# serval/kaboodle

Hardware: AMD Instinct MI355X
Metric: simulated peer-rounds/sec (whole node) + rounds to fingerprint convergence (higher is better)
Workload: dtype u8

## Files before the change

### include/kaboodle_sim.h

```cpp
#ifndef KABOODLE_SIM_H
#define KABOODLE_SIM_H

#include <stddef.h>
#include <stdint.h>

#ifdef __cplusplus
extern "C" {
#endif

#define KB_ABI_VERSION 3u

enum {
  KB_OK = 0,
  KB_INVALID_OPERATION = 1,
  KB_IO_ERROR = 2,
  KB_NO_DEVICE = 3,
  KB_STOPPING_FAILED = 4,
  KB_INVALID_ARGUMENT = 5,
  KB_CAPACITY = 6
};

enum { KB_INIT_JOIN = 0,
       KB_INIT_CONVERGED = 1 };

enum { KB_FAILED_SIM_SENDER = 0,
       KB_FAILED_SOCKET_FAITHFUL = 1 };

typedef struct kb_config {
  uint32_t abi_version;
  uint32_t capacity;
  uint32_t initial_nodes;
  uint32_t init_mode;
  uint64_t seed;
  uint32_t loss_threshold;
  uint32_t churn_threshold;
  int32_t  fault_end_round;
  uint32_t max_waves;
  uint32_t failed_mode;
  uint32_t id_len;
  uint32_t partition_groups;
  int32_t  partition_start;
  int32_t  partition_end;
  int32_t  device;
  uint32_t debug_flags;
  uint32_t track_latency;
  uint32_t variant;
  uint32_t sparse_row_cap;
  uint32_t stat_flags;
  uint32_t reserved[1];
} kb_config;
enum { KB_STAT_NO_SF_FAILED_DROPS = 1u };
enum { KB_VARIANT_SAME_WINDOW_BCAST = 1u,
       KB_VARIANT_EXACT_LRU = 2u,
       KB_VARIANT_SPARSE_ROWS = 4u };

enum {
  KB_DBG_PHASEB_HBM = 1u,
  KB_DBG_RESP_HBM = 2u,
  KB_DBG_KP_HBM = 4u,
  KB_DBG_KP_BIG_SMALL = 8u,
  KB_DBG_PROC_UNSORTED = 16u,
  KB_DBG_WAVE_GRAPH = 32u,
  KB_DBG_RESP_WAVE_HBM = 64u,
  KB_DBG_NO_UNION = 128u,
  KB_DBG_A3X_KPL8 = 256u,
  KB_DBG_A3X_WIDE = 512u,
  KB_DBG_WAVE0_SERIAL = 1024u,
  KB_DBG_RESP_SERIAL = 2048u
};

enum { KB_STATE_KNOWN = 0, KB_STATE_WAITING_FOR_PING = 1, KB_STATE_WAITING_FOR_INDIRECT_PING = 2 };
typedef struct kb_peer_state {
  uint32_t peer;
  uint32_t state;
  int32_t  since;
  uint32_t latency_ms;
  uint32_t identity_len;
  uint8_t  identity[32];
} kb_peer_state;
#define KB_LATENCY_NONE 0xFFFFFFFFu

typedef struct kb_stats {
  int32_t  round;
  uint32_t alive;
  uint32_t agree;
  int32_t  first_converged_round;
  int32_t  last_converged_round;
  uint32_t next_free_id;
  uint64_t sent_ping, sent_ping_req, sent_ack, sent_known_peers, sent_kpr;
  uint64_t bcast_join, bcast_failed;
  uint64_t drop_dead, drop_loss, drop_window, drop_oversize, drop_partition, drop_bcast;
  uint64_t removed_timeout, removed_failed, join_responses, curious_overflow, churn_leaves, churn_joins;
  uint64_t sent_kp_ids;
  uint64_t alive_rounds;
  uint64_t probe_responses;
  uint64_t exported;
  uint64_t reserved[4];
} kb_stats;

typedef struct kb_sim kb_sim;

void kb_config_default(kb_config* cfg);

int  kb_sim_create(const kb_config* cfg, kb_sim** out);
int  kb_sim_destroy(kb_sim* sim);
int  kb_sim_step(kb_sim* sim, uint32_t rounds);

int  kb_sim_start_node(kb_sim* sim, uint32_t node);
int  kb_sim_stop_node(kb_sim* sim, uint32_t node);
int  kb_sim_restart_node(kb_sim* sim, uint32_t node, uint32_t* new_node);
int  kb_sim_is_running(kb_sim* sim, uint32_t node, int* running);
int  kb_sim_ping_addrs(kb_sim* sim, uint32_t node, const uint32_t* peers, size_t n);
int  kb_sim_set_identity(kb_sim* sim, uint32_t node, const uint8_t* identity, size_t len);
int  kb_sim_identity(kb_sim* sim, uint32_t node, uint8_t* buf, size_t cap, size_t* len);

int  kb_sim_fingerprint(kb_sim* sim, uint32_t node, uint32_t* fp);
int  kb_sim_fingerprints(kb_sim* sim, uint32_t* fps, size_t cap);
int  kb_sim_peers(kb_sim* sim, uint32_t node, uint32_t* peers, size_t cap, size_t* n);
int  kb_sim_peer_states(kb_sim* sim, uint32_t node, kb_peer_state* out, size_t cap, size_t* n);
int  kb_sim_stats(kb_sim* sim, kb_stats* out);
int  kb_sim_true_fingerprint(kb_sim* sim, uint32_t* fp);
// ... 112 lines not shown
```

### kaboodle_amd/_ffi.py

```python
from __future__ import annotations

import ctypes as C
import os
from dataclasses import dataclass

KB_ABI_VERSION = 3
KB_OK, KB_INVALID_OPERATION, KB_IO_ERROR, KB_NO_DEVICE, KB_STOPPING_FAILED, KB_INVALID_ARGUMENT, KB_CAPACITY = range(7)
KB_INIT_JOIN, KB_INIT_CONVERGED = 0, 1
KB_FAILED_SIM_SENDER, KB_FAILED_SOCKET_FAITHFUL = 0, 1
KB_DBG_PHASEB_HBM, KB_DBG_RESP_HBM, KB_DBG_KP_HBM, KB_DBG_KP_BIG_SMALL, KB_DBG_PROC_UNSORTED = 1, 2, 4, 8, 16
KB_DBG_ALL = 31
KB_DBG_WAVE_GRAPH = 32
KB_DBG_RESP_WAVE_HBM = 64
KB_DBG_NO_UNION = 128
KB_DBG_A3X_KPL8 = 256
KB_DBG_A3X_WIDE = 512
KB_DBG_WAVE0_SERIAL = 1024
KB_DBG_RESP_SERIAL = 2048
KB_VARIANT_SAME_WINDOW_BCAST, KB_VARIANT_EXACT_LRU = 1, 2
KB_STAT_NO_SF_FAILED_DROPS = 1
KB_VARIANT_SPARSE_ROWS = 4
KB_LATENCY_NONE = 0xFFFFFFFF
KT_ROWPASS, KT_ROUND, KT_FOLD, KT_RESP, KT_PROC = 0, 1, 2, 3, 4
KB_WAVE_SLOTS = 9
STATE_NAMES = {0: "Known", 1: "WaitingForPing", 2: "WaitingForIndirectPing"}


class KbConfig(C.Structure):
    _fields_ = [
        ("abi_version", C.c_uint32), ("capacity", C.c_uint32), ("initial_nodes", C.c_uint32),
        ("init_mode", C.c_uint32), ("seed", C.c_uint64), ("loss_threshold", C.c_uint32),
        ("churn_threshold", C.c_uint32), ("fault_end_round", C.c_int32), ("max_waves", C.c_uint32),
        ("failed_mode", C.c_uint32), ("id_len", C.c_uint32), ("partition_groups", C.c_uint32),
        ("partition_start", C.c_int32), ("partition_end", C.c_int32), ("device", C.c_int32),
        ("debug_flags", C.c_uint32), ("track_latency", C.c_uint32), ("variant", C.c_uint32),
        ("sparse_row_cap", C.c_uint32), ("stat_flags", C.c_uint32), ("reserved", C.c_uint32 * 1),
    ]


class KbPeerState(C.Structure):
    _fields_ = [("peer", C.c_uint32), ("state", C.c_uint32), ("since", C.c_int32), ("latency_ms", C.c_uint32),
                ("identity_len", C.c_uint32), ("identity", C.c_uint8 * 32)]


PEER_STATE_DTYPE = [("peer", "<u4"), ("state", "<u4"), ("since", "<i4"), ("latency_ms", "<u4"), ("identity_len", "<u4"),
                    ("identity", "u1", (32,))]


class KbStats(C.Structure):
    _fields_ = [
        ("round", C.c_int32), ("alive", C.c_uint32), ("agree", C.c_uint32),
        ("first_converged_round", C.c_int32), ("last_converged_round", C.c_int32), ("next_free_id", C.c_uint32),
        ("sent_ping", C.c_uint64), ("sent_ping_req", C.c_uint64), ("sent_ack", C.c_uint64),
        ("sent_known_peers", C.c_uint64), ("sent_kpr", C.c_uint64),
        ("bcast_join", C.c_uint64), ("bcast_failed", C.c_uint64),
        ("drop_dead", C.c_uint64), ("drop_loss", C.c_uint64), ("drop_window", C.c_uint64),
        ("drop_oversize", C.c_uint64), ("drop_partition", C.c_uint64), ("drop_bcast", C.c_uint64),
        ("removed_timeout", C.c_uint64), ("removed_failed", C.c_uint64), ("join_responses", C.c_uint64),
        ("curious_overflow", C.c_uint64), ("churn_leaves", C.c_uint64), ("churn_joins", C.c_uint64),
        ("sent_kp_ids", C.c_uint64), ("alive_rounds", C.c_uint64), ("probe_responses", C.c_uint64),
        ("exported", C.c_uint64), ("reserved", C.c_uint64 * 4),
    ]

    def as_dict(self) -> dict:
        return {n: getattr(self, n) for n, _ in self._fields_ if n != "reserved"}


class KbKernelTime(C.Structure):
    _fields_ = [("name", C.c_char * 24), ("ms", C.c_double), ("launches", C.c_uint64), ("bytes", C.c_uint64),
                ("has_bytes", C.c_uint32), ("pad", C.c_uint32), ("wave_ms", C.c_double * KB_WAVE_SLOTS)]

# ... 927 lines not shown
```

### kaboodle_amd/csrc/kb_common.h

```cpp
#pragma once
#include "kb_device.h"
#include "../../include/kaboodle_sim.h"

namespace kb {

enum StatIdx {
  S_PING, S_PINGREQ, S_ACK, S_KP, S_KPR, S_BJOIN, S_BFAIL, S_DEAD, S_LOSS, S_WINDOW, S_OVERSIZE, S_PART, S_BDROP,
  S_RMTIMEOUT, S_RMFAILED, S_JRESP, S_CUROVF, S_CLEAVE, S_CJOIN,
  S_KPIDS,
  S_ROWB,
  S_FOLDB,
  S_A3ROWS, S_A3DEEP, S_A3CHUNKS,
  S_ALIVER,
  S_RESPB,
  S_PROCB,
  S_PROBERESP,
  S_EXPORT,
  S_A3X32, S_A3XCLAMP, S_A3XFEW, S_A3XLIVE, S_A3XWIDE,
  NSTAT
};
enum CtrIdx {
  C_KP, C_SLOW, C_ACTIVE, C_AGREE, C_ALIVE, C_LEAVES, C_NEXTFREE, C_ERR, C_FIRSTCONV, C_LASTCONV, C_LASTAGREE,
  C_LASTALIVE, C_DBG_INS, C_DBG_FP, C_DBG_MAXFP,
  C_DBG_KPR, C_DBG_KPRLOG, C_DBG_BASE,
  C_DBG_TNODE, C_DBG_TMAX, C_DBG_TBASE, C_DBG_TINS,
  C_DBG_TSTART, C_DBG_TEND, C_DBG_MSGS,
  C_TICK,
  C_ROUND,
  C_PATHS,
  C_DBG_SLOW_LONG, C_DBG_SLOW_NONMEM, C_DBG_SLOW_DIRTY, C_DBG_SLOW_KPR, C_DBG_SLOW_OTHER,
  C_RESTN,
  C_XREC, C_XPAY,
  NCTR
};
enum : uint32_t { PATH_PHASEB_HBM = 1, PATH_RESP_SCRATCH_SAMPLED = 2, PATH_RESP_SCRATCH_FULL = 4, PATH_KP_BIG_HBM = 8,
                  PATH_PROC_UNSORTED = 16, PATH_BFAIL_PREP_HBM = 32, PATH_RESP_WAVE = 64, PATH_KP_BIG_LDS = 128,
                  PATH_RESP_WAVE_HBM = 256,
                  PATH_PROC_DEFERRED = 512,
                  PATH_ROWPASS_LDS_HBM_LISTS = 1024,
                  PATH_KPR_WRAPPED = 2048,
                  PATH_RESP_JOINERS_HBM = 4096,
                  PATH_JOIN_LIST_PAST_UCAP = 8192,
                  PATH_RESP_PHASE1 = 16384,
                  PATH_A2_RESPONDER = 32768 };
constexpr int NSEG = 64;
constexpr int ZT = 9;
constexpr int ZB = 9 * 1024;

struct Dev {
  uint32_t lo, hi;
  uint32_t C, W, SEGW, NWR;
  uint32_t segq, segm;
  uint32_t k0, k1;
  uint32_t loss_thr, churn_thr;
  int32_t fault_end;
  uint32_t failed_mode;
  uint32_t pgroups;
  int32_t pstart, pend;
  uint32_t uniform, L;
  uint32_t capk, capj;
  uint32_t paybound;
  uint32_t dbg;
  uint32_t dev;
  uint8_t* stamp;
  uint32_t* bits;
  uint2* segp;
  unsigned long long* sdirty;
  uint8_t* dirty;
  uint8_t* alive;
  uint8_t* idset;
  uint32_t* abits;
  int32_t* start_round;
  uint32_t* n;
  uint32_t* fp;
  int32_t* last_bcast;
  uint32_t* a3cur;
  Susp* susp;
  Cur* cur;
  uint32_t* paq;
  uint32_t* paq_n;
  uint32_t* cseg;
  uint32_t* segmul;
  uint32_t* seglen;
  uint32_t* zpow;
  uint32_t* zfin;
// ... 379 lines not shown
```

### kaboodle_amd/csrc/kb_sim.hip

```cpp
#include <hip/hip_runtime.h>
#include <hip/hip_ext.h>
#include <stdint.h>
#include <stdio.h>
#include <string.h>
#include <stdlib.h>
#include <string>
#include <vector>
#include <array>
#include <algorithm>
#include <atomic>
#include <thread>
#include "kb_common.h"
#include "kb_wire.h"
#include "kb_round.h"
#include "kb_tick.h"
#include "kb_waves.h"
#include "kb_xfer.h"
#include "kb_sparse.h"

using namespace kb;

enum KId : int {
  KI_REBASE, KI_EVENTS, KI_CHURN_LEAVE, KI_CHURN_JOIN, KI_ALIVE_BITS, KI_TRUEFP_PART, KI_TRUEFP_FIN, KI_LOG_MARK,
  KI_LAT_MARK, KI_BFAIL_PREP, KI_ROWPASS, KI_LAT_SWEEP, KI_SCAN_TILES, KI_SCAN_APPLY, KI_SET_CAP, KI_RESP_WAVE,
// ... 266 lines not shown

struct kb_sim {
  kb_config cfg;
  SpSim* sp = nullptr;
  Dev d;
  int device;
  hipStream_t st;
  hipStream_t st2 = nullptr;
  hipStream_t st3 = nullptr;
  hipEvent_t ev_fork[5] = {nullptr, nullptr, nullptr, nullptr, nullptr}, ev_join[5] = {nullptr, nullptr, nullptr, nullptr, nullptr};
  uint32_t C, W, S;
  uint32_t lo, hi, R;
  int rank, world;
  Xfer* xf;
  bool in_group;
  std::vector<void*> allocs;
  int32_t round;
  bool probed = false;
  std::vector<uint8_t> h_ident, h_idlen;
  std::vector<uint8_t> h_pend; std::vector<int16_t> h_pendlen;
  std::vector<uint8_t> h_moved;
  std::vector<uint8_t> h_idset;
  std::vector<uint8_t> h_ext;
  size_t n_ext = 0;
  std::vector<XRec> inj; std::vector<uint32_t> inj_ids;
  std::vector<uint32_t> inj_join;
  XRec* d_inj = nullptr; uint32_t* d_inj_ids = nullptr; size_t d_inj_cap = 0, d_inj_ids_cap = 0;
  std::vector<kb_unicast> xq; std::vector<uint32_t> xq_ids;
  std::vector<Event> events;
  uint32_t* rpack = nullptr; uint32_t* rpack_in = nullptr;
  std::vector<kb_wire_addr> probe_q, probes;
  std::vector<kb_probe_response> presp;
  uint2* d_presp = nullptr; uint32_t* d_presp_n = nullptr; size_t presp_cap = 0;
  OutBuf ob[2];
  WaveCtl wc;
  uint32_t msg_cap, pay_cap;
  BCast* bfail; BCast* bjoin;
  BCast* bfail_loc; BCast* bjoin_loc;
  uint32_t nf, nj;
  uint32_t ucap = 0;
  uint32_t host_paths = 0;
  uint64_t xbytes_cross = 0, xbytes_all = 0;
  BcastSlots bs;
  uint32_t* join_off; uint32_t* fail_off;
  uint32_t* scan_tot; uint32_t* scan_tiles;
  unsigned long long* newmask; unsigned long long* respmask; size_t mask_words;
  unsigned long long* newmask_base; unsigned long long* respmask_base;
  uint32_t* nresp; uint32_t* paysum; uint32_t* nbase; uint32_t* resp_off;
  uint32_t* resp_nodes; uint32_t* bf_gid; uint8_t* bf_dep;
  uint32_t* slow;
  uint32_t* rest[2] = {nullptr, nullptr};
  uint32_t* rest2n = nullptr;
  uint8_t* a2flag = nullptr;
  uint32_t* defer = nullptr;
  uint32_t* w0ctr = nullptr;
  uint16_t* lat_col;
  uint32_t* fnamed;
  uint32_t* resp_scratch; size_t resp_scratch_words;
  RowOut ro;
  Event* d_events; size_t events_cap;
  XState xs;
  uint32_t* xall; unsigned long long* xstats;
  std::vector<uint32_t> h_xall;
  Msg* rmsg; uint32_t* rpay; uint8_t* rstatus; uint32_t* rinbox; uint32_t* rkp;
  size_t rmsg_cap, rpay_cap;
  double round_ms;
  uint32_t* rr = nullptr;
  uint64_t round_launches, bj_total, bf_total;
  struct KRec { int16_t kid, wave; hipEvent_t a, b; };
  int prof_level = 1;
  bool capturing = false;
  int cur_wave = -1;
  std::vector<hipEvent_t> ev_free;
  std::vector<KRec> krec;
  double k_ms[NKI] = {};
  double k_wms[NKI][KB_WAVE_SLOTS] = {};
  uint64_t k_n[NKI] = {};
  uint64_t k_bytes0[NSTAT] = {};
  uint64_t host_syncs = 0;
  uint32_t ncu = 256;
  uint32_t* cs_buf = nullptr;
  uint32_t* rc_buf = nullptr;
  uint2* rc_pairs = nullptr; size_t rc_pairs_cap = 0;
  char* fc_buf = nullptr; size_t fc_cap = 0;
  double census_ms[CM_N] = {};
  bool debug_waves = false;
  size_t lds_per_cu = 65536;
  std::vector<kb_sim*> shards;
  LocalHub* hub;
  std::vector<uint32_t> watch_node, watch_fp;
  std::vector<uint32_t*> watch_snap;
  uint32_t* ev_out = nullptr;
  uint32_t* h_pin = nullptr;
  uint32_t* d_pin = nullptr;
  uint32_t pin_seq = 0;
  uint64_t occ_key = ~0ull; int occ_val = 0;
  bool graph_on = false;
  hipGraph_t wave_graph = nullptr; hipGraphExec_t wave_exec = nullptr;
  uint64_t buf_gen = 0, wave_gen = ~0ull;
  uint32_t* lc_buf = nullptr;
  double sn_ms = 0;
  uint32_t* dl_base = nullptr;
  uint8_t* dl_run = nullptr;
  int32_t dl_round = 0;
  uint32_t* dl_buf = nullptr;
  uint32_t* is_buf = nullptr;
// ... 220 lines not shown
constexpr uint32_t KB_FOLD_WAVES = 16384;
  while (S < 64 && groups * S < KB_FOLD_WAVES) S <<= 1;
  s->S = S;
  Dev& d = s->d;
  d.lo = s->lo; d.hi = s->hi;
  d.C = C; d.W = W; d.SEGW = W / NSEG; d.NWR = W / 32;
  d.segq = d.SEGW / 128;
  d.segm = d.segq > 1 ? (uint32_t)(((1ull << 32) + d.segq - 1) / d.segq) : 0u;
  d.k0 = (uint32_t)cfg->seed; d.k1 = (uint32_t)(cfg->seed >> 32);
  d.loss_thr = cfg->loss_threshold; d.churn_thr = cfg->churn_threshold; d.fault_end = cfg->fault_end_round;
  d.failed_mode = cfg->failed_mode; d.pgroups = cfg->partition_groups; d.pstart = cfg->partition_start;
  d.pend = cfg->partition_end;
  const uint32_t Lid = cfg->id_len;
  d.capk = (BUFSZ - 20 - Lid) / (18 + Lid);
  d.capj = (BUFSZ - 20 - Lid - 1) / (18 + Lid);
  d.paybound = C < d.capk ? C : d.capk;
  d.dbg = cfg->debug_flags;
  if (const char* dv = getenv("KB_DEV")) d.dev = (uint32_t)atoi(dv);
  s->debug_waves = getenv("KB_DEBUG_WAVES") != nullptr;
  if (const char* gv = getenv("KB_WAVE_GRAPH")) s->graph_on = atoi(gv) != 0;
  if (cfg->debug_flags & KB_DBG_WAVE_GRAPH) s->graph_on = true;
  s->h_ident.assign((size_t)C * MAXID, 0); s->h_idlen.assign(C, (uint8_t)Lid);
  s->h_pend.assign((size_t)C * MAXID, 0); s->h_pendlen.assign(C, (int16_t)-1); s->h_moved.assign(C, 0);
  s->h_idset.assign(C, 0);
  for (uint32_t j = 0; j < C; ++j) default_identity(j, Lid, &s->h_ident[(size_t)j * MAXID]);
  hipError_t e = hipSuccess;
#define A(ptr, n) if (e == hipSuccess) e = talloc(s, &(ptr), (n))
#define AR(ptr, n) if (e == hipSuccess) e = ralloc(s, &(ptr), (n))
  AR(d.stamp, W); AR(d.bits, d.NWR); AR(d.segp, NSEG); AR(d.sdirty, 1);
  AR(d.dirty, 1); A(d.alive, C); A(d.idset, C); A(d.ext, C); A(d.abits, d.NWR); A(d.start_round, C); AR(d.n, 1); AR(d.fp, 1);
  AR(d.last_bcast, 1); AR(d.a3cur, 1); AR(d.susp, SLOTS); AR(d.cur, CSLOTS); AR(d.paq, PAQ);
  AR(d.paq_n, 1); A(d.cseg, C); A(d.segmul, C); A(d.seglen, C); A(d.zpow, (size_t)C + 2); A(d.zfin, (size_t)C + 2);
  A(d.ztab, 17 * 128); A(d.zbtab, ZB);
  A(d.htab, (size_t)(W / 8) * 256); A(d.stats, NSTAT); A(d.sacc, (size_t)NACC * NSTAT); A(d.ctr, NCTR); A(d.truefp, 1); A(d.tfpart, TRUEFP_G);
  AR(d.flog, LOGCAP); AR(d.flog_n, 1); AR(d.fstart, 16); AR(d.kpr_big, 1);
  if (cfg->variant == KB_VARIANT_EXACT_LRU) { AR(d.tst, W); AR(d.tlb, W / 1024); }
  if (cfg->track_latency) { A(d.lat, (size_t)W * lat_stride(R)); A(s->lat_col, C); A(s->fnamed, d.NWR); }
  s->msg_cap = std::max<uint32_t>(8u * R + (uint32_t)TICK_MAX * R, 1u << 16);
  s->pay_cap = std::max<uint32_t>((d.capk + 1) * R, 1u << 24);
  for (int b = 0; b < 2; ++b) {
    A(s->ob[b].msgs, s->msg_cap); A(s->ob[b].pay, s->pay_cap); AR(s->ob[b].off, 1); AR(s->ob[b].cap, 1);
    AR(s->ob[b].cnt, 1); AR(s->ob[b].poff, 1);
    s->ob[b].msg_cap = s->msg_cap; s->ob[b].pay_cap = s->pay_cap;
  }
  AR(s->wc.cnt1, 1); AR(s->wc.bnd, 1); AR(s->wc.bpay, 1); AR(s->wc.cursor, 1);
  AR(s->wc.in_off, 1); A(s->wc.active, R);
  AR(s->wc.kcnt, 1); AR(s->wc.kpay, 1); AR(s->wc.kcur, 1); AR(s->wc.koff, 1);
  if (!xf) { A(s->wc.status, s->msg_cap); A(s->wc.inbox, s->msg_cap); A(s->wc.kin, s->msg_cap); }
  A(s->bfail, (size_t)C * SLOTS); A(s->bjoin, C);
  AR(s->bs.join, 1); AR(s->bs.nfail, 1); AR(s->bs.fail, SLOTS); AR(s->join_off, 1); AR(s->fail_off, 1);
  A(s->scan_tot, 32); A(s->rr, 4); A(s->scan_tiles, 5 * ((std::max<size_t>(C, (size_t)world * R) + 1023) / 1024) + 5);
  AR(s->nresp, 1); AR(s->paysum, 1); AR(s->nbase, 1); AR(s->resp_off, 1);
  A(s->resp_nodes, R); A(s->bf_gid, (size_t)C * SLOTS); A(s->bf_dep, (size_t)C * SLOTS); A(s->slow, R); A(s->defer, R); A(s->w0ctr, W0_WORDS);
  A(s->rest[0], R); A(s->rest[1], R); A(s->rest2n, 1); AR(s->a2flag, 1);
  AR(s->ro.part, 10);
  if (xf) {
    XState& x = s->xs;
    x.world = (uint32_t)world; x.R = R; x.S = rows_per; x.RS = R + 1;
    x.NWW = d.NWR; x.nju = 0; x.nj = 0; x.uon = 0;
    s->ucap = std::min<uint32_t>(UCAP, C);
    A(x.ostatus, s->msg_cap); A(x.xcnt, (size_t)world * x.RS); A(x.xpay, (size_t)world * x.RS);
    A(x.xoff, (size_t)world * x.RS); A(x.xpoff, (size_t)world * x.RS); A(x.xb, 2 * world);
    A(x.smsg, (size_t)s->msg_cap + s->ucap); A(x.spay, (size_t)s->pay_cap + (size_t)s->ucap * x.NWW);
    A(x.jslot, C); A(x.ubits, (size_t)s->ucap * x.NWW); A(x.uany, s->ucap);
    A(s->xall, std::max(2 * world * world, 3 * world));
    A(s->xstats, NSTAT);
    A(s->bfail_loc, (size_t)R * SLOTS); A(s->bjoin_loc, R);
    s->h_xall.assign(2 * world * world, 0);
  }
#undef A
#undef AR
  if (e != hipSuccess) { seterr(std::string("device allocation failed: ") + hipGetErrorString(e)); destroy_shard(s); return KB_CAPACITY; }
  (void)hipMemset(L(s, d.kpr_big), 0xFF, 4ull * R);
  if (xf) { (void)hipMemset(s->xs.jslot, 0xFF, 4ull * C); (void)hipMemset(s->xs.ubits, 0, 4ull * s->ucap * s->xs.NWW); }
  if (d.lat) { (void)hipMemset(d.lat, 0xFF, 2ull * lat_stride(R) * W); (void)hipMemset(s->fnamed, 0, 4ull * d.NWR); }
  if (d.tst) {
    (void)hipMemsetD32(d.tst + (size_t)s->lo * W, INT32_MIN / 2, (size_t)R * W);
    (void)hipMemsetD32(d.tlb + (size_t)s->lo * (W / 1024), INT32_MIN, (size_t)R * (W / 1024));
  }
  s->wc.msg_cap = s->msg_cap; s->wc.pay_cap = s->pay_cap;
  if (hipStreamCreateWithFlags(&s->st, hipStreamNonBlocking) != hipSuccess) { destroy_shard(s); seterr("stream"); return KB_IO_ERROR; }
  if (hipStreamCreateWithFlags(&s->st2, hipStreamNonBlocking) != hipSuccess) { destroy_shard(s); seterr("stream"); return KB_IO_ERROR; }
  if (hipStreamCreateWithFlags(&s->st3, hipStreamNonBlocking) != hipSuccess) { destroy_shard(s); seterr("stream"); return KB_IO_ERROR; }
  for (int k = 0; k < 5; ++k)
    if (hipEventCreateWithFlags(&s->ev_fork[k], hipEventDisableTiming) != hipSuccess ||
        hipEventCreateWithFlags(&s->ev_join[k], hipEventDisableTiming) != hipSuccess) { destroy_shard(s); seterr("events"); return KB_IO_ERROR; }
  if (hipHostMalloc((void**)&s->h_pin, 4 * PIN_WORDS, hipHostMallocMapped | hipHostMallocCoherent) != hipSuccess) {
    s->h_pin = nullptr; destroy_shard(s); seterr("pinned buffer"); return KB_IO_ERROR;
  }
  if (hipHostGetDevicePointer((void**)&s->d_pin, s->h_pin, 0) != hipSuccess) { destroy_shard(s); seterr("pinned buffer mapping"); return KB_IO_ERROR; }
  if (const char* pv = getenv("KB_PROF")) s->prof_level = atoi(pv);
  int rc = upload_segments(s);
  if (rc) { destroy_shard(s); return rc; }
  uint32_t ctr0[NCTR] = {0};
  ctr0[C_NEXTFREE] = cfg->initial_nodes;
  ctr0[C_FIRSTCONV] = 0xFFFFFFFFu; ctr0[C_LASTCONV] = 0xFFFFFFFFu;
  if (hipMemcpy(d.ctr, ctr0, sizeof ctr0, hipMemcpyHostToDevice) != hipSuccess) { destroy_shard(s); seterr("ctr upload"); return KB_IO_ERROR; }
  const uint32_t tb = 256, gb = (C + tb - 1) / tb;
  if (cfg->init_mode == KB_INIT_CONVERGED) {
    k_init_converged_rows<<<4096, 256, 0, s->st>>>(d, cfg->initial_nodes);
    k_init_converged_nodes<<<gb, tb, 0, s->st>>>(d, cfg->initial_nodes);
  } else {
    k_init_nodes<<<gb, tb, 0, s->st>>>(d, cfg->initial_nodes);
  }
  if (hipStreamSynchronize(s->st) != hipSuccess) { destroy_shard(s); seterr("init failed"); return KB_IO_ERROR; }
  *out = s;
  return KB_OK;
// ... 489 lines not shown
  const uint32_t R = s->R;
  if (!s->inj_join.empty()) { const int rc = merge_ext_joins(s->st, s->bjoin, &s->nj, s->inj_join, 0, s->C); if (rc) return rc; }
  PhaseB& pb = q.pb;
  pb.bfail = s->bfail; pb.nf = s->nf; pb.bjoin = s->bjoin; pb.nj = s->nj; pb.JW = (s->nj + 63) / 64;
  pb.nresp = s->nresp; pb.paysum = s->paysum; pb.nbase = s->nbase;
  if (pb.JW) {
    const size_t words = (size_t)R * pb.JW;
    if (words > s->mask_words) {
      const int rc = eng_grow_group(s, &s->mask_words, words, words, &s->newmask_base, &s->respmask_base);
      if (rc) return rc;
    }
    s->newmask = bias(s->newmask_base, pb.JW, s->lo);
    s->respmask = bias(s->respmask_base, pb.JW, s->lo);
  }
  pb.newmask = s->newmask; pb.respmask = s->respmask;
  pb.gid = s->bf_gid; pb.dep = s->bf_dep;
  q.lat_fail = d.lat && s->nf && d.failed_mode == KB_FAILED_SIM_SENDER;
  pb.fnamed = q.lat_fail ? s->fnamed : nullptr;
  if (q.lat_fail) klaunch(s, KI_LAT_MARK, k_lat_mark, dim3((s->nf + 255) / 256), dim3(256), 0, (const BCast*)s->bfail, s->nf, s->fnamed);
  const bool pb_hbm = (d.dbg & KB_DBG_PHASEB_HBM) != 0;
  if (s->nf > BFAIL_LDS_MAX || (pb_hbm && s->nf)) klaunch(s, KI_BFAIL_PREP, k_bfail_prep, dim3((s->nf + 255) / 256), dim3(256), 0, (const BCast*)s->bfail, s->nf, s->bf_gid, s->bf_dep, d.ctr + C_PATHS);
  else if (s->nf) klaunch(s, KI_BFAIL_PREP, k_bfail_prep_lds, dim3(1), dim3(1024), 0, (const BCast*)s->bfail, s->nf, s->bf_gid, s->bf_dep);
  { const int rc = dbg_bcast_shape(s, r); if (rc) return rc; }
  {
    const RowPlan p = rowpass_plan(s, pb_hbm);
    { const int rc = dbg_rowpass_begin(s, r, p); if (rc) return rc; }
    if (p.ldsb && !p.ll) s->host_paths |= PATH_ROWPASS_LDS_HBM_LISTS;
    rowpass_with(p, [&](auto k) { klaunch(s, KI_ROWPASS, k, dim3(p.blocks), dim3(64 * p.wpb), (uint32_t)p.lds, d, pb, s->ro, r); });
    { const int rc = dbg_rowpass_shares(s, r, p); if (rc) return rc; }
  }
  side_fork(s, 0);
  klaunch_on(s, s->st2, KI_ALIVE_BITS, k_alive_bits, dim3((d.NWR + TB - 1) / TB), dim3(TB), 0, d);
  klaunch_on(s, s->st2, KI_TRUEFP_PART, k_truefp_part, dim3(TRUEFP_G), dim3(256), 0, d, d.tfpart);
  klaunch_on(s, s->st2, KI_TRUEFP_FIN, k_truefp_fin, dim3(1), dim3(64), 0, d, d.tfpart);
  side_done(s, 0);
  if (q.lat_fail) {
    klaunch_on(s, s->st2, KI_LAT_SWEEP, k_lat_sweep, dim3((lat_stride(R) / 8 + 255) / 256, std::min<uint32_t>(s->nf, 16384)), dim3(256), 0, d,
            (const BCast*)s->bfail, (const uint32_t*)s->bf_gid, s->nf, s->fnamed);
    side_done(s, 1);
  }
  { const int rc = round_take_probes(s, R, &q.np); if (rc) return rc; }
  if (q.np) klaunch(s, KI_PROBE, k_probe, dim3(gnode(s)), dim3(TB), 0, d, q.np, r, s->d_presp, s->d_presp_n, (uint32_t)s->presp_cap);
  return KB_OK;
}

static bool resp_rows_hbm(const kb_sim* s) { return s->W > RESP_LDS_W || (s->d.dbg & KB_DBG_RESP_HBM); }
static int launch_join_responses(kb_sim* s, Round& q, uint32_t resp_nodes, uint32_t phase) {
  Dev& d = s->d;
  const int32_t r = q.r;
  OutBuf& o0 = s->ob[0];
  hipStream_t st = phase == 2 ? s->st3 : s->st;
  uint32_t* rest = s->rest[phase == 2];
  uint32_t* restn = phase == 2 ? s->rest2n : d.ctr + C_RESTN;
  const uint32_t wcap = phase == 1 ? s->ncu : 4096;
  const uint32_t grid = std::min<uint32_t>(resp_nodes, 4096);
  const size_t words = resp_words(d.NWR, s->W / 256);
  uint32_t* scratch = nullptr;
  size_t lds = 4 * words;
  const bool resp_hbm = resp_rows_hbm(s);
  if (resp_hbm) {
    { const int rc = eng_grow(s, &s->resp_scratch, &s->resp_scratch_words, words * grid); if (rc) return rc; }
    scratch = s->resp_scratch;
    lds = 0;
  }
  const size_t wlds = 16ull * rwave_words(d.NWR, s->W / 256);
  const size_t hlds = 4ull * rwave_head(s->W / 256);
  const bool full_on = wlds <= 65536 && !(d.dbg & (KB_DBG_RESP_HBM | KB_DBG_RESP_WAVE_HBM));
  const uint32_t hwaves = (uint32_t)std::min<size_t>(4, 65536 / hlds);
  const bool head_on = !full_on && hwaves >= 1 && !(d.dbg & KB_DBG_RESP_HBM);
  const bool wave_on = full_on || head_on;
  { const int rc = dbg_resp_clear(s); if (rc) return rc; }
  if (full_on) {
    klaunch_on(s, st, KI_RESP_WAVE, k_resp_wave<false>, dim3(std::min<uint32_t>((resp_nodes + 3) / 4, wcap)), dim3(256), (uint32_t)wlds, d,
               q.pb, (const uint32_t*)s->resp_nodes, (const uint32_t*)(s->scan_tot + 4), o0, r, rest, restn, phase, (const uint8_t*)s->a2flag);
  } else if (head_on) {
    klaunch_on(s, st, KI_RESP_WAVE, k_resp_wave<true>, dim3(std::min<uint32_t>((resp_nodes + hwaves - 1) / hwaves, wcap)),
               dim3(64 * hwaves), (uint32_t)(hwaves * hlds), d, q.pb, (const uint32_t*)s->resp_nodes,
               (const uint32_t*)(s->scan_tot + 4), o0, r, rest, restn, phase, (const uint8_t*)s->a2flag);
  }
  klaunch_on(s, st, KI_RESP_NODE, k_resp_node, dim3(wave_on ? std::min<uint32_t>(grid, 2 * s->ncu) : grid), dim3(256), (uint32_t)lds, d, q.pb,
             (const uint32_t*)(wave_on ? rest : s->resp_nodes), (const uint32_t*)(wave_on ? restn : s->scan_tot + 4),
             o0, r, scratch, wave_on, phase, (const uint8_t*)s->a2flag);
  return dbg_resp_report(s, r);
}
static bool resp_overlap_on(const kb_sim* s) {
  return !s->xf && !resp_rows_hbm(s) && !s->debug_waves && !(s->d.dbg & KB_DBG_RESP_SERIAL);
}
static void launch_tick_scan(kb_sim* s, Round& q) {
  klaunch(s, KI_TICK_SCAN, k_tick_scan, dim3(gnode(s)), dim3(TB), 0, s->d, s->bs, q.r, s->slow, s->a2flag);
  q.tick_scanned = true;
}

static int round_wave0_regions(kb_sim* s, Round& q) {
  Dev& d = s->d;
  const int32_t r = q.r;
  const uint32_t R = s->R;
  OutBuf& o0 = s->ob[0];
  q.ninj = (uint32_t)s->inj.size();
  if (q.ninj) {
    if (q.ninj > s->d_inj_cap) { const int rc = eng_grow(s, &s->d_inj, &s->d_inj_cap, 2 * (size_t)q.ninj); if (rc) return rc; }
    if (s->inj_ids.size() > s->d_inj_ids_cap || !s->d_inj_ids) {
      const int rc = eng_grow(s, &s->d_inj_ids, &s->d_inj_ids_cap, 2 * s->inj_ids.size() + 16);
      if (rc) return rc;
    }
    HIPCHK(hipMemcpyAsync(s->d_inj, s->inj.data(), sizeof(XRec) * q.ninj, hipMemcpyHostToDevice, s->st));
    if (!s->inj_ids.empty()) {
      HIPCHK(hipMemcpyAsync(s->d_inj_ids, s->inj_ids.data(), 4 * s->inj_ids.size(), hipMemcpyHostToDevice, s->st));
      q.inj_pay = true;
    }
    klaunch(s, KI_EVENTS, k_inject_prep, dim3(1), dim3(64), 0, d, (const XRec*)s->d_inj, q.ninj, s->paysum);
  }
  {
    ScanArgs a = scan_args(s, R, s->scan_tot);
    a.narr = 3;
    a.in[0] = L(s, s->nresp); a.out[0] = L(s, s->resp_off);
    a.in[1] = L(s, s->paysum); a.out[1] = L(s, o0.poff);
    a.in[2] = L(s, s->nresp); a.out[2] = L(s, o0.off); a.addc[2] = TICK_MAX;
    a.list = s->resp_nodes; a.list_base = s->lo;
    launch_scan(s, a);
  }
  const bool need_tot = s->nj > 0 || q.inj_pay;
  klaunch(s, KI_SET_CAP, k_set_cap, dim3(gnode(s)), dim3(TB), 0, d, s->nresp, o0.cap, o0.cnt, s->scan_tot, s->d_pin, need_tot ? ++s->pin_seq : 0u,
          s->rest2n);
  if (!need_tot) return KB_OK;
  const uint32_t* tot = s->h_pin;
  { const int rc = wait_pin(s, s->pin_seq); if (rc) return rc; }
  const uint32_t pay_tot = tot[1], msg_tot = tot[2], resp_nodes = tot[4];
  if (msg_tot > o0.msg_cap || pay_tot > o0.pay_cap) { const int rc = grow_wave0(s, msg_tot, pay_tot); if (rc) return rc; }
  if (s->n_ext) { const int rc = round_size_exports(s, msg_tot, pay_tot); if (rc) return rc; }
  if (!resp_nodes) return KB_OK;
  if (!resp_overlap_on(s)) return launch_join_responses(s, q, resp_nodes, 0);
  launch_tick_scan(s, q);
  side_fork(s, 4);
  { const int rc = launch_join_responses(s, q, resp_nodes, 2); if (rc) return rc; }
  side_done(s, 4);
  q.resp_side = true;
  return launch_join_responses(s, q, resp_nodes, 1);
}

static int round_tick(kb_sim* s, Round& q) {
  Dev& d = s->d;
  const int32_t r = q.r;
  const uint32_t R = s->R, gn = gnode(s);
  OutBuf& o0 = s->ob[0];
  if (q.lat_fail) side_join(s, 1);
  if (!q.tick_scanned) launch_tick_scan(s, q);
  klaunch(s, KI_TICK_PRE, k_tick_pre, dim3(std::min<uint32_t>((R + 3) / 4, 1024)), dim3(256), 0, d, o0, s->bs, r, s->slow,
          (const uint32_t*)s->nresp);
  if (d.tst) {
    side_fork(s, 2);
    const uint32_t kpl = a3_kpl(s->W, d.dbg);
    if (kpl == 2) klaunch_on(s, s->st2, KI_A3_EXACT, k_a3_exact<2>, dim3((R + 3) / 4), dim3(256), 0, d, s->ro.part, r);
    else if (kpl) klaunch_on(s, s->st2, KI_A3_EXACT, k_a3_exact<A3X_KPL>, dim3((R + 3) / 4), dim3(256), 0, d, s->ro.part, r);
    else klaunch_on(s, s->st2, KI_A3_EXACT, k_a3_exact<0>, dim3((R + 3) / 4), dim3(256), 0, d, s->ro.part, r);
    side_done(s, 2);
  }
  if (d.uniform) klaunch(s, KI_FOLD, k_fold, dim3(((R + 63) / 64 + 3) / 4 * s->S), dim3(256), 0, d, FoldArgs{s->S});
  if (d.uniform) klaunch(s, KI_FP_ROWS, k_fp_rows, dim3((FP_LANES * R + TB - 1) / TB), dim3(TB), 0, d);
  side_join(s, 0);
  if (d.tst) side_join(s, 2);
  if (q.resp_side) side_join(s, 4);
  klaunch(s, KI_TICK_POST, k_tick_post, dim3(gn), dim3(TB), 0, d, s->ro, o0, r);
  if (q.ninj) {
    klaunch(s, KI_EVENTS, k_inject, dim3(1), dim3(64), 0, d, o0, (const XRec*)s->d_inj, q.ninj, (const uint32_t*)s->d_inj_ids);
    s->inj.clear(); s->inj_ids.clear();
  }
  {
    ScanArgs a = scan_args(s, R, s->scan_tot);
    a.narr = 2;
    a.in[0] = L(s, s->bs.join); a.out[0] = L(s, s->join_off);
    a.in[1] = L(s, s->bs.nfail); a.out[1] = L(s, s->fail_off);
    launch_scan(s, a);
  }
  klaunch(s, KI_BCAST_WRITE, k_bcast_write, dim3(gn), dim3(TB), 0, d, s->bs, (const uint32_t*)s->join_off,
          (const uint32_t*)s->fail_off, s->xf ? s->bjoin_loc : s->bjoin, s->xf ? s->bfail_loc : s->bfail);
  return KB_OK;
}

static int round_window(kb_sim* s, Round& q) {
  hipStream_t st = s->st;
  if (s->xf || s->debug_waves || !s->graph_on) return launch_waves(s, q.r);
  if (!s->wave_exec || s->wave_gen != s->buf_gen) {
    if (s->wave_exec) { (void)hipGraphExecDestroy(s->wave_exec); s->wave_exec = nullptr; }
    if (s->wave_graph) { (void)hipGraphDestroy(s->wave_graph); s->wave_graph = nullptr; }
    HIPCHK(hipStreamBeginCapture(st, hipStreamCaptureModeThreadLocal));
    s->capturing = true;
    const int rc = launch_waves(s, -1);
    s->capturing = false;
    hipGraph_t g = nullptr;
    const hipError_t e = hipStreamEndCapture(st, &g);
// ... 667 lines not shown
```

### kaboodle_amd/csrc/kb_tick.h

```cpp
#pragma once
#include "kb_common.h"

namespace kb {

struct BcastSlots { uint32_t* join; uint32_t* nfail; uint32_t* fail; };

__device__ __attribute__((always_inline)) inline void tick_a2(const Dev& d, const OutBuf& ob, const BcastSlots& bs, int32_t r,
                                                              uint32_t i, uint32_t l, uint32_t* pr, uint32_t* pp,
                                                              uint32_t* pid, const uint32_t* nresp) {
  uint32_t n = d.n[i];
  Susp* sl = d.susp + (size_t)i * SLOTS;
  const Susp me = l < SLOTS ? sl[l] : Susp{0, 0, 0, 0};
  const bool occ = l < SLOTS && me.kind != 0;
  const unsigned long long occm = __ballot(occ);
  const unsigned long long tim = __ballot(occ && r - me.since >= PING_TIMEOUT);
  if (!tim) { if (l == 0) bs.nfail[i] = 0; return; }
  const uint32_t nsusp = __popcll(occm);
  const uint32_t m = n - 1 - nsusp;
  uint32_t myrank = 0;
  for (int k = 0; k < SLOTS; ++k) if (((occm >> k) & 1ull) && rdl(me.peer, k) < me.peer) myrank++;
  uint32_t npick = 0, nind = 0, nrem = 0;
  uint32_t indirect[SLOTS], removed[SLOTS];
  for (uint32_t t = 0; t < nsusp; ++t) {
    const unsigned long long who = __ballot(occ && myrank == t);
// ... 43 lines not shown
#pragma unroll
      for (int u = 0; u < PB; ++u) {
        if (base > maxrank) break;
        const uint32_t w = w0 + 64u * u + l, id0 = w * 128;
        const uint32_t wd[4] = {v[u].x, v[u].y, v[u].z, v[u].w};
        uint32_t c = __popc(wd[0]) + __popc(wd[1]) + __popc(wd[2]) + __popc(wd[3]);
#pragma unroll
        for (int k = 0; k <= SLOTS; ++k) c -= (ex[k] - id0 < 128u) ? 1u : 0u;
        const uint32_t exl = wave_excl(c), tot = wave_sum(c);
        for (uint32_t q = 0; q < npick; ++q) {
          const uint32_t rk = pr[q];
          if (rk >= base + exl && rk < base + exl + c) {
            uint32_t rem = rk - base - exl, id = 0xFFFFFFFFu;
#pragma unroll
            for (int k = 0; k < 4; ++k) {
              uint32_t m = wd[k];
#pragma unroll
              for (int e = 0; e <= SLOTS; ++e) if ((ex[e] >> 5) == w * 4 + k) m &= ~(1u << (ex[e] & 31));
              const uint32_t pc = __popc(m);
              if (id == 0xFFFFFFFFu) { if (rem < pc) id = id0 + 32 * k + select_in_word(m, rem); else rem -= pc; }
            }
            pid[q] = id;
          }
        }
        base += tot;
      }
    }
    wait_lds();
    __builtin_amdgcn_wave_barrier();
    for (uint32_t q = 0; q < npick; ++q) emit_msg(ob, d, i, oseq, pid[q], K_PINGREQ, pp[q], 0, 0, 0);
  }
  if (l == 0) {
    for (uint32_t q = 0; q < nind; ++q)
      for (int k = 0; k < SLOTS; ++k) if (sl[k].kind && sl[k].peer == indirect[q]) { sl[k].kind = SK_WFIP; sl[k].since = r; }
    Cur* cu = d.cur + (size_t)i * CSLOTS;
    unsigned long long segs = 0;
    for (uint32_t q = 0; q < nrem; ++q) {
      const uint32_t p = removed[q];
      susp_clear(d, i, p);
      mem_clr(d, i, p);
      lat_none(d, i, p);
      segs |= seg_bit(d, p);
      n--;
      for (int c = 0; c < CSLOTS; ++c) if (cu[c].used && cu[c].peer == p) cu[c].used = 0;
      bs.fail[(size_t)i * SLOTS + q] = p;
    }
    bs.nfail[i] = nrem;
    if (nrem) { d.n[i] = n; mark(d, i, segs); slot_add(d, S_RMTIMEOUT, nrem); }
    if (nrem && nresp[i]) path_hit(d, PATH_A2_RESPONDER);
    ob.cnt[i] = oseq;
  }
}

__global__ __launch_bounds__(256) void k_tick_scan(Dev d, BcastSlots bs, int32_t r, uint32_t* list, uint8_t* a2flag) {
  const uint32_t i = d.lo + blockIdx.x * blockDim.x + threadIdx.x;
  if (i >= d.hi) return;
  a2flag[i] = 0;
  if (!d.alive[i]) { bs.join[i] = 0; bs.nfail[i] = 0; return; }
  const int32_t lb = d.last_bcast[i];
  uint32_t j = 0;
  if (lb == NONE_ROUND || (r - lb >= REBROADCAST && d.n[i] <= 1)) { j = 1; d.last_bcast[i] = r; }
  bs.join[i] = j;
  const Susp* sl = d.susp + (size_t)i * SLOTS;
  bool tim = false;
#pragma unroll
  for (int k = 0; k < SLOTS; ++k) { const Susp x = sl[k]; tim |= x.kind != 0 && r - x.since >= PING_TIMEOUT; }
  if (!tim) { bs.nfail[i] = 0; return; }
  const unsigned long long m = __ballot(true);
  const int first = __ffsll((long long)m) - 1;
  uint32_t base = 0;
  if (lane() == (uint32_t)first) base = atomicAdd(&d.ctr[C_TICK], (uint32_t)__popcll(m));
  list[rdl(base, first) + __popcll(m & ((1ull << lane()) - 1ull))] = i;
  a2flag[i] = 1;
}

__global__ __launch_bounds__(256) void k_tick_pre(Dev d, OutBuf ob, BcastSlots bs, int32_t r, const uint32_t* list,
                                                  const uint32_t* nresp) {
  __shared__ uint32_t s_pick_rank[4][SLOTS * 3], s_pick_peer[4][SLOTS * 3], s_pick_id[4][SLOTS * 3];
  const uint32_t wv = threadIdx.x >> 6;
  const uint32_t l = lane();
  const uint32_t nlist = d.ctr[C_TICK];
  for (uint32_t it = blockIdx.x * 4 + wv; it < nlist; it += gridDim.x * 4) {
    tick_a2(d, ob, bs, r, list[it], l, s_pick_rank[wv], s_pick_peer[wv], s_pick_id[wv], nresp);
  }
}


struct FoldArgs { uint32_t S; };

__global__ __launch_bounds__(256) void k_fold(Dev d, FoldArgs fa) {
  __shared__ uint32_t zb[ZB];
  load_zbtab(d, zb);
  const uint32_t S = fa.S;
  const uint32_t s = blockIdx.x % S;
  const uint32_t g = (blockIdx.x / S) * 4 + (threadIdx.x >> 6);
  const uint32_t i0 = d.lo + g * 64 + lane();
  const bool act = i0 < d.hi && d.alive[i0] && d.uniform;
  const unsigned long long actm = __ballot(act);
  __shared__ uint32_t s_nb[4];
  uint32_t nbytes = 0;
  if (actm) {
    const uint32_t i = act ? i0 : d.lo + g * 64 + (uint32_t)(__ffsll((long long)actm) - 1);
    const uint32_t* bw = bits_of(d, i);
    const uint32_t spp = NSEG / S;
    const unsigned long long sd = act ? d.sdirty[i] : 0ull;
    unsigned long long folded = 0;
    for (uint32_t k = s * spp; k < (s + 1) * spp; ++k) {
      const bool mine = (sd >> k) & 1ull;
      if (!__ballot(mine)) continue;
      const uint32_t c0 = k * d.SEGW, c1 = c0 + d.SEGW;
      uint32_t raw = 0, cnt = 0;
      uint4 mb = *reinterpret_cast<const uint4*>(bw + (c0 >> 5));
      for (uint32_t col = c0; col < c1; col += 128) {
        const uint32_t mw[4] = {mb.x, mb.y, mb.z, mb.w};
        uint32_t hv[16];
        const uint32_t* ht = d.htab + (size_t)(col >> 3) * 256;
#pragma unroll
        for (int h = 0; h < 16; ++h) hv[h] = ht[h * 256 + ((mw[h >> 2] >> (8 * (h & 3))) & 0xFFu)];
        if (col + 128 < c1) mb = *reinterpret_cast<const uint4*>(bw + ((col + 128) >> 5));
#pragma unroll
        for (int h = 0; h < 16; ++h) {
          const uint32_t c = __popc((mw[h >> 2] >> (8 * (h & 3))) & 0xFFu);
          raw = mulzb(zb, raw, c) ^ hv[h];
          cnt += c;
        }
      }
// ... 88 lines not shown
      oseq++;
    }
    d.paq_n[i] = 0;
    ob.cnt[i] = oseq;
    thread_refresh_fp(d, i);
    agree = d.fp[i] == d.truefp[0];
  }
  const unsigned long long t = block_sum(agree);
  if (threadIdx.x == 0 && t) atomicAdd(&d.ctr[C_AGREE], (uint32_t)t);
}

__global__ void k_bcast_write(Dev d, BcastSlots bs, const uint32_t* join_off, const uint32_t* fail_off, BCast* bjoin,
                              BCast* bfail) {
  const uint32_t i = d.lo + blockIdx.x * blockDim.x + threadIdx.x;
  if (i >= d.hi) return;
  uint32_t bseq = 0;
  if (bs.join[i]) bjoin[join_off[i]] = BCast{i, i, bseq++, 0};
  const uint32_t nfl = bs.nfail[i];
  for (uint32_t q = 0; q < nfl; ++q) bfail[fail_off[i] + q] = BCast{i, bs.fail[(size_t)i * SLOTS + q], bseq++, 0};
}

__global__ void k_inject_prep(Dev d, const XRec* inj, uint32_t n, uint32_t* paysum) {
  if (threadIdx.x || blockIdx.x) return;
  for (uint32_t k = 0; k < n; ++k)
    if (local(d, inj[k].sender) && inj[k].kind == K_KP) paysum[inj[k].sender] += inj[k].pay_len;
}
__global__ void k_inject(Dev d, OutBuf ob, const XRec* inj, uint32_t n, const uint32_t* ids) {
  if (threadIdx.x || blockIdx.x) return;
  for (uint32_t k = 0; k < n; ++k) {
    const XRec x = inj[k];
    if (!local(d, x.sender)) continue;
    const uint32_t slot = ob.cnt[x.sender];
    if (slot >= ob.cap[x.sender]) { set_err(d, DERR_OUTBOX); continue; }
    const uint32_t off = ob.poff[x.sender] + x.pad;
    if (x.kind == K_KP) for (uint32_t q = 0; q < x.pay_len; ++q) ob.pay[off + q] = ids[x.pay_off + q];
    ob.msgs[ob.off[x.sender] + slot] = Msg{x.dest, x.sender, slot, x.kind, x.kind == K_KP ? x.pay_len : x.a, x.fp, x.n,
                                           x.kind == K_KP ? off : 0u};
    ob.cnt[x.sender] = slot + 1;
  }
}

__global__ void k_round_end(Dev d, int32_t r, const uint32_t* tot, uint32_t* rres, uint32_t seq, uint32_t* rr) {
  if (threadIdx.x || blockIdx.x) return;
  const uint32_t a = d.ctr[C_AGREE], al = d.ctr[C_ALIVE];
  d.ctr[C_LASTAGREE] = a; d.ctr[C_LASTALIVE] = al;
  if (d.lo == 0) d.stats[S_ALIVER] += al;
  const uint32_t v[3] = {tot[0], tot[1], d.ctr[C_ERR]};
  rr[0] = v[0]; rr[1] = v[1]; rr[2] = v[2];
  if (seq) pin_publish(rres, v, 3, seq);
  if (al && a == al) {
    if ((int32_t)d.ctr[C_FIRSTCONV] < 0) d.ctr[C_FIRSTCONV] = (uint32_t)r;
    d.ctr[C_LASTCONV] = (uint32_t)r;
  }
  d.ctr[C_AGREE] = 0; d.ctr[C_ALIVE] = 0; d.ctr[C_TICK] = 0;
}

}
```

Before: 13.13 million.

## Compact phase-1 join-response nodes in tick scan instead of scanning all responders

The tick-scan kernel now also builds a compacted list of nodes that have both timed-out suspects and pending join responses, counted under a new C_RESP1 counter. The phase-1 response kernels read this smaller list instead of the full responder list, so they do less redundant per-node work. A debug flag and a device bit add options to run phase 1 on a single workgroup or before the side-stream phase 2. The cost is an extra ballot and atomic in tick scan, one more buffer, and a counter reset at round end.

```diff
diff --git a/include/kaboodle_sim.h b/include/kaboodle_sim.h
--- a/include/kaboodle_sim.h
+++ b/include/kaboodle_sim.h
@@ -66,7 +66,8 @@
   KB_DBG_A3X_KPL8 = 256u,
   KB_DBG_A3X_WIDE = 512u,
   KB_DBG_WAVE0_SERIAL = 1024u,
-  KB_DBG_RESP_SERIAL = 2048u
+  KB_DBG_RESP_SERIAL = 2048u,
+  KB_DBG_RESP1_ONE_WG = 4096u
 };
 
 enum { KB_STATE_KNOWN = 0, KB_STATE_WAITING_FOR_PING = 1, KB_STATE_WAITING_FOR_INDIRECT_PING = 2 };
diff --git a/kaboodle_amd/_ffi.py b/kaboodle_amd/_ffi.py
--- a/kaboodle_amd/_ffi.py
+++ b/kaboodle_amd/_ffi.py
@@ -17,6 +17,7 @@
 KB_DBG_A3X_WIDE = 512
 KB_DBG_WAVE0_SERIAL = 1024
 KB_DBG_RESP_SERIAL = 2048
+KB_DBG_RESP1_ONE_WG = 4096
 KB_VARIANT_SAME_WINDOW_BCAST, KB_VARIANT_EXACT_LRU = 1, 2
 KB_STAT_NO_SF_FAILED_DROPS = 1
 KB_VARIANT_SPARSE_ROWS = 4
diff --git a/kaboodle_amd/csrc/kb_common.h b/kaboodle_amd/csrc/kb_common.h
--- a/kaboodle_amd/csrc/kb_common.h
+++ b/kaboodle_amd/csrc/kb_common.h
@@ -31,6 +31,7 @@
   C_DBG_SLOW_LONG, C_DBG_SLOW_NONMEM, C_DBG_SLOW_DIRTY, C_DBG_SLOW_KPR, C_DBG_SLOW_OTHER,
   C_RESTN,
   C_XREC, C_XPAY,
+  C_RESP1,
   NCTR
 };
 enum : uint32_t { PATH_PHASEB_HBM = 1, PATH_RESP_SCRATCH_SAMPLED = 2, PATH_RESP_SCRATCH_FULL = 4, PATH_KP_BIG_HBM = 8,
diff --git a/kaboodle_amd/csrc/kb_sim.hip b/kaboodle_amd/csrc/kb_sim.hip
--- a/kaboodle_amd/csrc/kb_sim.hip
+++ b/kaboodle_amd/csrc/kb_sim.hip
@@ -342,6 +342,7 @@
   uint32_t* rest[2] = {nullptr, nullptr};
   uint32_t* rest2n = nullptr;
   uint8_t* a2flag = nullptr;
+  uint32_t* resp1 = nullptr;
   uint32_t* defer = nullptr;
   uint32_t* w0ctr = nullptr;
   uint16_t* lat_col;
@@ -668,7 +669,7 @@
   A(s->scan_tot, 32); A(s->rr, 4); A(s->scan_tiles, 5 * ((std::max<size_t>(C, (size_t)world * R) + 1023) / 1024) + 5);
   AR(s->nresp, 1); AR(s->paysum, 1); AR(s->nbase, 1); AR(s->resp_off, 1);
   A(s->resp_nodes, R); A(s->bf_gid, (size_t)C * SLOTS); A(s->bf_dep, (size_t)C * SLOTS); A(s->slow, R); A(s->defer, R); A(s->w0ctr, W0_WORDS);
-  A(s->rest[0], R); A(s->rest[1], R); A(s->rest2n, 1); AR(s->a2flag, 1);
+  A(s->rest[0], R); A(s->rest[1], R); A(s->rest2n, 1); AR(s->a2flag, 1); A(s->resp1, R);
   AR(s->ro.part, 10);
   if (xf) {
     XState& x = s->xs;
@@ -1264,8 +1265,11 @@
   hipStream_t st = phase == 2 ? s->st3 : s->st;
   uint32_t* rest = s->rest[phase == 2];
   uint32_t* restn = phase == 2 ? s->rest2n : d.ctr + C_RESTN;
-  const uint32_t wcap = phase == 1 ? s->ncu : 4096;
-  const uint32_t grid = std::min<uint32_t>(resp_nodes, 4096);
+  const bool one_wg = phase == 1 && (d.dbg & KB_DBG_RESP1_ONE_WG);
+  const uint32_t wcap = one_wg ? 1u : phase == 1 ? s->ncu : 4096;
+  const uint32_t grid = one_wg ? 1u : std::min<uint32_t>(resp_nodes, 4096);
+  const uint32_t* nodes = phase == 1 ? s->resp1 : s->resp_nodes;
+  const uint32_t* nnodes_p = phase == 1 ? d.ctr + C_RESP1 : s->scan_tot + 4;
   const size_t words = resp_words(d.NWR, s->W / 256);
   uint32_t* scratch = nullptr;
   size_t lds = 4 * words;
@@ -1284,14 +1288,14 @@
   { const int rc = dbg_resp_clear(s); if (rc) return rc; }
   if (full_on) {
     klaunch_on(s, st, KI_RESP_WAVE, k_resp_wave<false>, dim3(std::min<uint32_t>((resp_nodes + 3) / 4, wcap)), dim3(256), (uint32_t)wlds, d,
-               q.pb, (const uint32_t*)s->resp_nodes, (const uint32_t*)(s->scan_tot + 4), o0, r, rest, restn, phase, (const uint8_t*)s->a2flag);
+               q.pb, nodes, nnodes_p, o0, r, rest, restn, phase, (const uint8_t*)s->a2flag);
   } else if (head_on) {
     klaunch_on(s, st, KI_RESP_WAVE, k_resp_wave<true>, dim3(std::min<uint32_t>((resp_nodes + hwaves - 1) / hwaves, wcap)),
-               dim3(64 * hwaves), (uint32_t)(hwaves * hlds), d, q.pb, (const uint32_t*)s->resp_nodes,
-               (const uint32_t*)(s->scan_tot + 4), o0, r, rest, restn, phase, (const uint8_t*)s->a2flag);
+               dim3(64 * hwaves), (uint32_t)(hwaves * hlds), d, q.pb, nodes, nnodes_p, o0, r, rest, restn, phase,
+               (const uint8_t*)s->a2flag);
   }
   klaunch_on(s, st, KI_RESP_NODE, k_resp_node, dim3(wave_on ? std::min<uint32_t>(grid, 2 * s->ncu) : grid), dim3(256), (uint32_t)lds, d, q.pb,
-             (const uint32_t*)(wave_on ? rest : s->resp_nodes), (const uint32_t*)(wave_on ? restn : s->scan_tot + 4),
+             wave_on ? (const uint32_t*)rest : nodes, wave_on ? (const uint32_t*)restn : nnodes_p,
              o0, r, scratch, wave_on, phase, (const uint8_t*)s->a2flag);
   return dbg_resp_report(s, r);
 }
@@ -1299,7 +1303,9 @@
   return !s->xf && !resp_rows_hbm(s) && !s->debug_waves && !(s->d.dbg & KB_DBG_RESP_SERIAL);
 }
 static void launch_tick_scan(kb_sim* s, Round& q) {
-  klaunch(s, KI_TICK_SCAN, k_tick_scan, dim3(gnode(s)), dim3(TB), 0, s->d, s->bs, q.r, s->slow, s->a2flag);
+  const bool on = resp_overlap_on(s);
+  klaunch(s, KI_TICK_SCAN, k_tick_scan, dim3(gnode(s)), dim3(TB), 0, s->d, s->bs, q.r, s->slow, s->a2flag,
+          on ? (const uint32_t*)s->nresp : (const uint32_t*)nullptr, on ? s->resp1 : (uint32_t*)nullptr);
   q.tick_scanned = true;
 }
 
@@ -1343,11 +1349,13 @@
   if (!resp_nodes) return KB_OK;
   if (!resp_overlap_on(s)) return launch_join_responses(s, q, resp_nodes, 0);
   launch_tick_scan(s, q);
+  const bool p1_first = (d.dev & 8192) != 0;
+  if (p1_first) { const int rc = launch_join_responses(s, q, resp_nodes, 1); if (rc) return rc; }
   side_fork(s, 4);
   { const int rc = launch_join_responses(s, q, resp_nodes, 2); if (rc) return rc; }
   side_done(s, 4);
   q.resp_side = true;
-  return launch_join_responses(s, q, resp_nodes, 1);
+  return p1_first ? KB_OK : launch_join_responses(s, q, resp_nodes, 1);
 }
 
 static int round_tick(kb_sim* s, Round& q) {
diff --git a/kaboodle_amd/csrc/kb_tick.h b/kaboodle_amd/csrc/kb_tick.h
--- a/kaboodle_amd/csrc/kb_tick.h
+++ b/kaboodle_amd/csrc/kb_tick.h
@@ -119,7 +119,8 @@
   }
 }
 
-__global__ __launch_bounds__(256) void k_tick_scan(Dev d, BcastSlots bs, int32_t r, uint32_t* list, uint8_t* a2flag) {
+__global__ __launch_bounds__(256) void k_tick_scan(Dev d, BcastSlots bs, int32_t r, uint32_t* list, uint8_t* a2flag,
+                                                   const uint32_t* nresp, uint32_t* resp1) {
   const uint32_t i = d.lo + blockIdx.x * blockDim.x + threadIdx.x;
   if (i >= d.hi) return;
   a2flag[i] = 0;
@@ -139,6 +140,14 @@
   if (lane() == (uint32_t)first) base = atomicAdd(&d.ctr[C_TICK], (uint32_t)__popcll(m));
   list[rdl(base, first) + __popcll(m & ((1ull << lane()) - 1ull))] = i;
   a2flag[i] = 1;
+  if (!resp1) return;
+  const bool resp = nresp[i] > 0;
+  const unsigned long long m1 = __ballot(resp);
+  if (!m1) return;
+  uint32_t base1 = 0;
+  if (lane() == (uint32_t)first) base1 = atomicAdd(&d.ctr[C_RESP1], (uint32_t)__popcll(m1));
+  base1 = rdl(base1, first);
+  if (resp) resp1[base1 + __popcll(m1 & ((1ull << lane()) - 1ull))] = i;
 }
 
 __global__ __launch_bounds__(256) void k_tick_pre(Dev d, OutBuf ob, BcastSlots bs, int32_t r, const uint32_t* list,
@@ -333,7 +342,7 @@
     if ((int32_t)d.ctr[C_FIRSTCONV] < 0) d.ctr[C_FIRSTCONV] = (uint32_t)r;
     d.ctr[C_LASTCONV] = (uint32_t)r;
   }
-  d.ctr[C_AGREE] = 0; d.ctr[C_ALIVE] = 0; d.ctr[C_TICK] = 0;
-}
-
-}
+  d.ctr[C_AGREE] = 0; d.ctr[C_ALIVE] = 0; d.ctr[C_TICK] = 0; d.ctr[C_RESP1] = 0;
+}
+
+}
```

After: 13.19 million (median of 3 runs). Within noise of the previous version (+0.4%).
